# Luca96/carla-driving-rl-agent

Measured on AMD Instinct MI355X. Metric: PPO update-steps/sec (batch=256, 4x90x120x3 obs), higher is better.
Workload: dtype f32; 1 GPU; configs[1]: synthetic rollout buffer 256x4-frame 90x120x3 obs per GPU, full CARLANetwork fwd/bwd + PPO (re-sampled Beta, pathwise) / value loss + clip + Adam, fp32; per_gpu_batch=256, global_batch=256, parallelism=dp1, policy_loss=resampled (reference-faithful)

## Files before the change

carla-driving-rl-agent_amd/csrc/gemm_tn_lds.hip:

```cpp
#include <stdlib.h>

#include "colreduce.h"
#include "mfma_x3.h"

namespace cdrl {

struct TnLdsArgs {
    View A, D;
    float* part;
    int M, N, K, G, Mg;
    int rows_per, nspg;
    const float* a_stats;
    TnBnBwd db;
};

constexpr int TNL_R = 32;

template <int MODE, bool APRO, bool DPRO>
__global__ void __launch_bounds__(256, 2) tn_lds_kernel(TnLdsArgs a) {
    constexpr bool BH = MODE == 2, F32 = MODE == 0, X3 = MODE == 3;
    constexpr int NBUF = X3 ? 1 : 2, PL = X3 ? 3 : 1;
    constexpr int TNL_CS = F32 ? TNL_R + 1 : TNL_R / 2 + 1;
    __shared__ uint32_t AsT[NBUF * PL][128 * TNL_CS];
    __shared__ uint32_t DsT[NBUF * PL][128 * TNL_CS];
    constexpr uint32_t ESZ = BH ? 2u : 4u;
    const int tid = threadIdx.x, lane = tid & 63, wave = tid >> 6;
    const int l32 = lane & 31, lh = lane >> 5;
    const int K = a.K, N = a.N;
    const int k0 = blockIdx.y * 128, n0 = blockIdx.z * 128;
    const int KT = min(4, (K - k0 + 31) / 32), NT = min(4, (N - n0 + 31) / 32);
    const int grp = blockIdx.x / a.nspg;
    const int64_t gend = (int64_t)(grp + 1) * a.Mg;
    const int64_t mbeg64 = (int64_t)grp * a.Mg + (int64_t)(blockIdx.x % a.nspg) * a.rows_per;
    const int mb = (int)mbeg64;
    const int me = (int)min(mbeg64 + a.rows_per, gend);
    const int rg = tid >> 5, cq = tid & 31;
    const int ka = k0 + 4 * cq, nd = n0 + 4 * cq;
    float asc[4], ash[4], qm[4], qi[4], qsc[4], qsh[4], qk1[4], qk2[4], qk3[4];
#pragma unroll
    for (int j = 0; j < 4; ++j) {
        asc[j] = 1.0f;
        ash[j] = 0.0f;
        if (APRO) {
            const bool on = ka + j < K;
            asc[j] = on ? a.a_stats[2 * a.G * K + grp * K + ka + j] : 0.0f;
            ash[j] = on ? a.a_stats[3 * a.G * K + grp * K + ka + j] : 0.0f;
        }
        qm[j] = qi[j] = qsc[j] = qsh[j] = qk1[j] = qk2[j] = qk3[j] = 0.0f;
        if (DPRO && nd + j < N) {
            const int GN = a.G * N, o = grp * N + nd + j;
            qm[j] = a.db.stats[0 * GN + o];
            qi[j] = a.db.stats[1 * GN + o];
            qsc[j] = a.db.stats[2 * GN + o];
            qsh[j] = a.db.stats[3 * GN + o];
            qk1[j] = a.db.coef[0 * GN + o];
            qk2[j] = a.db.coef[1 * GN + o];
            qk3[j] = a.db.coef[2 * GN + o];
        }
    }
    const bool relu = DPRO && a.db.act == ACT_RELU6;
    const __amdgpu_buffer_rsrc_t rA = buffer_rsrc(a.A.p, (int)((int64_t)a.M * a.A.ld * ESZ));
    const __amdgpu_buffer_rsrc_t rD = buffer_rsrc(a.D.p, (int)((int64_t)a.M * a.D.ld * ESZ));
    const __amdgpu_buffer_rsrc_t rY = buffer_rsrc(DPRO ? a.db.y : a.D.p, (int)((int64_t)a.M * (DPRO ? N : a.D.ld) * ESZ));
    const bool a4 = (ka + 3 < K);
    const bool a2 = (ka + 1 < K);
    const bool d4 = (nd + 3 < N), d2 = (nd + 1 < N);
    const int shuf = DPRO ? a.db.shuffle_ctot : 0;
    uint32_t voA = a2 ? (uint32_t)(a.A.coff + ka) * ESZ : OOR;
    uint32_t voD0, voD1;
    const bool dhalf = shuf && d2 && !d4;
    if (shuf) {
        voD0 = d2 ? (uint32_t)(shuffle_dst(a.D.coff + nd, shuf) - (dhalf ? 1 : 0)) * ESZ : OOR;
        voD1 = d2 ? (uint32_t)(shuffle_dst(a.D.coff + nd + 1, shuf) - (dhalf ? 1 : 0)) * ESZ : OOR;
    } else {
        voD0 = d2 ? (uint32_t)(a.D.coff + nd) * ESZ : OOR;
        voD1 = d4 ? (uint32_t)(a.D.coff + nd + 2) * ESZ : OOR;
    }
    const uint32_t voY = d2 ? (uint32_t)nd * ESZ : OOR;
    const uint32_t sA = (uint32_t)a.A.ld * ESZ, sD = (uint32_t)a.D.ld * ESZ, sY = (uint32_t)N * ESZ;
    auto ld2 = [&](const __amdgpu_buffer_rsrc_t& rs, uint32_t vo, uint32_t ro, float& x0, float& x1) {
        const uint32_t off = (vo & OOR) ? OOR : vo + ro;
        if (BH) {
            const uint32_t w = __builtin_amdgcn_raw_buffer_load_b32(rs, off, 0, 0);
            x0 = bf_lo(w);
            x1 = bf_hi(w);
        } else {
            const u32x2_t w = __builtin_amdgcn_raw_buffer_load_b64(rs, off, 0, 0);
            x0 = __uint_as_float(w[0]);
            x1 = __uint_as_float(w[1]);
        }
    };
    struct Regs {
        float a[4][4], d[4][4], y[DPRO ? 4 : 1][DPRO ? 4 : 1];
    };
    auto load_chunk = [&](int m0, Regs& r) {
#pragma unroll
        for (int i = 0; i < 4; ++i) {
            const int m = m0 + 4 * rg + i;
            const uint32_t msk = m < me ? 0u : OOR;
            const uint32_t row = (uint32_t)m;
            ld2(rA, voA | msk, row * sA, r.a[i][0], r.a[i][1]);
            ld2(rA, (a4 ? voA + 2 * ESZ : OOR) | msk, row * sA, r.a[i][2], r.a[i][3]);
            if (shuf) {
                ld2(rD, voD0 | msk, row * sD, r.d[i][0], r.d[i][2]);
                ld2(rD, voD1 | msk, row * sD, r.d[i][1], r.d[i][3]);
                if (dhalf) {
                    r.d[i][0] = r.d[i][2];
                    r.d[i][1] = r.d[i][3];
                    r.d[i][2] = r.d[i][3] = 0.0f;
                }
            } else {
                ld2(rD, voD0 | msk, row * sD, r.d[i][0], r.d[i][1]);
                ld2(rD, voD1 | msk, row * sD, r.d[i][2], r.d[i][3]);
            }
            if (DPRO) {
                ld2(rY, voY | msk, row * sY, r.y[DPRO ? i : 0][0], r.y[DPRO ? i : 0][DPRO ? 1 : 0]);
                ld2(rY, (d4 ? voY + 2 * ESZ : OOR) | msk, row * sY, r.y[DPRO ? i : 0][DPRO ? 2 : 0], r.y[DPRO ? i : 0][DPRO ? 3 : 0]);
            }
        }
        __builtin_amdgcn_sched_barrier(0);
    };
    auto store_chunk = [&](int m0, int buf, const Regs& r) {
        float keep[4];
#pragma unroll
        for (int i = 0; i < 4; ++i) keep[i] = (m0 + 4 * rg + i) < me ? 1.0f : 0.0f;
#pragma unroll
        for (int j = 0; j < 4; ++j) {
            float x[4], d[4];
#pragma unroll
            for (int i = 0; i < 4; ++i) {
                x[i] = r.a[i][j];
                if (APRO) x[i] = fmaf(asc[j], x[i], ash[j]);
                d[i] = r.d[i][j];
                if (DPRO) {
                    const float y = r.y[DPRO ? i : 0][DPRO ? j : 0];
                    if (relu) {
                        const float z = fmaf(qsc[j], y, qsh[j]);
                        d[i] = relu6_open(z) ? d[i] : 0.0f;
                    }
                    const float xh = (y - qm[j]) * qi[j];
                    d[i] = keep[i] * (qk1[j] * (d[i] - qk2[j] - xh * qk3[j]));
                }
            }
            const int c = 4 * cq + j;
            if (F32) {
                uint32_t* pa = &AsT[buf][c * TNL_CS + 4 * rg];
                uint32_t* pd = &DsT[buf][c * TNL_CS + 4 * rg];
#pragma unroll
                for (int i = 0; i < 4; ++i) {
                    pa[i] = __float_as_uint(x[i]);
                    pd[i] = __float_as_uint(d[i]);
                }
            } else if (X3) {
#pragma unroll
                for (int pl = 0; pl < 3; ++pl) {
                    float hx[4], hd[4];
#pragma unroll
                    for (int i = 0; i < 4; ++i) {
                        hx[i] = (float)(bf16_t)x[i];
                        hd[i] = (float)(bf16_t)d[i];
                        x[i] -= hx[i];
                        d[i] -= hd[i];
                    }
                    uint32_t* pa = &AsT[pl][c * TNL_CS + 2 * rg];
                    pa[0] = bf_pack(hx[0], hx[1]);
                    pa[1] = bf_pack(hx[2], hx[3]);
                    uint32_t* pd = &DsT[pl][c * TNL_CS + 2 * rg];
                    pd[0] = bf_pack(hd[0], hd[1]);
                    pd[1] = bf_pack(hd[2], hd[3]);
                }
            } else {
                uint32_t* pa = &AsT[buf][c * TNL_CS + 2 * rg];
                pa[0] = bf_pack(x[0], x[1]);
                pa[1] = bf_pack(x[2], x[3]);
                uint32_t* pd = &DsT[buf][c * TNL_CS + 2 * rg];
                pd[0] = bf_pack(d[0], d[1]);
                pd[1] = bf_pack(d[2], d[3]);
            }
        }
    };
    f32x16 acc[4];
#pragma unroll
    for (int j = 0; j < 4; ++j)
#pragma unroll
        for (int q = 0; q < 16; ++q) acc[j][q] = 0.0f;
    auto frag = [&](const uint32_t* base, int col, int s) -> bf16x8 {
        const uint32_t* p = base + col * TNL_CS + 8 * s + 4 * lh;
        u32x4_t w;
        w[0] = p[0];
        w[1] = p[1];
        w[2] = p[2];
        w[3] = p[3];
        return __builtin_bit_cast(bf16x8, w);
    };
    auto mma_chunk = [&](int buf) {
        if (wave >= KT) return;
        if (F32) {
            const uint32_t* pa = &AsT[buf][(wave * 32 + l32) * TNL_CS + lh];
#pragma unroll
            for (int s = 0; s < TNL_R / 2; ++s) {
                const float av = __uint_as_float(pa[2 * s]);
#pragma unroll
                for (int j = 0; j < 4; ++j) {
                    if (j < NT) {
                        const float dv = __uint_as_float(DsT[buf][(j * 32 + l32) * TNL_CS + 2 * s + lh]);
                        acc[j] = __builtin_amdgcn_mfma_f32_32x32x2f32(av, dv, acc[j], 0, 0, 0);
                    }
                }
            }
            return;
        }
        if (X3) {
#pragma unroll
            for (int s = 0; s < TNL_R / 16; ++s) {
                const bf16x8 a1 = frag(AsT[0], wave * 32 + l32, s), a2 = frag(AsT[X3 ? 1 : 0], wave * 32 + l32, s),
                             a3 = frag(AsT[X3 ? 2 : 0], wave * 32 + l32, s);
#pragma unroll
                for (int j = 0; j < 4; ++j) {
                    if (j < NT) {
                        const bf16x8 d1 = frag(DsT[0], j * 32 + l32, s), d2 = frag(DsT[X3 ? 1 : 0], j * 32 + l32, s),
                                     d3 = frag(DsT[X3 ? 2 : 0], j * 32 + l32, s);
                        acc[j] = __builtin_amdgcn_mfma_f32_32x32x16_bf16(a2, d2, acc[j], 0, 0, 0);
                        acc[j] = __builtin_amdgcn_mfma_f32_32x32x16_bf16(a3, d1, acc[j], 0, 0, 0);
                        acc[j] = __builtin_amdgcn_mfma_f32_32x32x16_bf16(a1, d3, acc[j], 0, 0, 0);
                        acc[j] = __builtin_amdgcn_mfma_f32_32x32x16_bf16(a2, d1, acc[j], 0, 0, 0);
                        acc[j] = __builtin_amdgcn_mfma_f32_32x32x16_bf16(a1, d2, acc[j], 0, 0, 0);
                        acc[j] = __builtin_amdgcn_mfma_f32_32x32x16_bf16(a1, d1, acc[j], 0, 0, 0);
                    }
                }
            }
            return;
        }
#pragma unroll
        for (int s = 0; s < TNL_R / 16; ++s) {
            const bf16x8 af = frag(AsT[buf], wave * 32 + l32, s);
#pragma unroll
            for (int j = 0; j < 4; ++j) {
                if (j < NT) {
                    const bf16x8 df = frag(DsT[buf], j * 32 + l32, s);
                    acc[j] = __builtin_amdgcn_mfma_f32_32x32x16_bf16(af, df, acc[j], 0, 0, 0);
                }
            }
        }
    };
    Regs r0;
    int c = 0;
    if (mb < me) load_chunk(mb, r0);
    for (int m0 = mb; m0 < me; m0 += TNL_R, ++c) {
        store_chunk(m0, X3 ? 0 : (c & 1), r0);
        __syncthreads();
        if (m0 + TNL_R < me) load_chunk(m0 + TNL_R, r0);
        mma_chunk(X3 ? 0 : (c & 1));
        if (X3) __syncthreads();
    }
    if (wave >= KT) return;
    float* out = a.part + (int64_t)blockIdx.x * K * N;
#pragma unroll
    for (int j = 0; j < 4; ++j) {
        const int n = n0 + j * 32 + l32;
        if (j >= NT || n >= N) continue;
#pragma unroll
        for (int q = 0; q < 16; ++q) {
            const int kk = acc_row(k0 + wave * 32, q, lh);
            if (kk < K) out[(int64_t)kk * N + n] = acc[j][q];
        }
    }
}

struct TnlPlan {
    int gy, gz, nspg, nsplit, rows_per;
};

static TnlPlan tnl_plan(int M, int N, int K, int G) {
    TnlPlan p;
    p.gy = cdiv(K, 128);
    p.gz = cdiv(N, 128);
    const int Mg = M / G;
    static const int wgs = 384;
    int target = wgs / (p.gy * p.gz * G);
    if (target < 1) target = 1;
    int ns = Mg / 128;
    if (ns > target) ns = target;
    if (ns < 1) ns = 1;
    p.rows_per = cdiv(cdiv(Mg, ns), TNL_R) * TNL_R;
    p.nspg = cdiv(Mg, p.rows_per);
    p.nsplit = G * p.nspg;
    return p;
}

int64_t gemm_tn_lds_part_elems(int M, int N, int K, int G) { return (int64_t)tnl_plan(M, N, K, G).nsplit * K * N; }

bool gemm_tn_lds_supported(View A, View D, int N, int K, int shuffle_ctot) {
    if ((A.ld & 1) || (A.coff & 1) || (D.ld & 1) || (D.coff & 1) || (K & 1) || (N & 1)) return false;
    if (shuffle_ctot && ((shuffle_ctot >> 1) & 1)) return false;
    return true;
}

void gemm_tn_lds_plan(TnPlan& p, int M, int N, int K, int G, int shuffle_ctot) {
    const TnlPlan q = tnl_plan(M, N, K, G);
    p.kernel = 2;
    p.NJW = p.WK = p.NSPL = p.RS = p.RS2 = p.U = 0;
    p.gy = q.gy;
    p.gz = q.gz;
    p.nspg = q.nspg;
    p.nsplit = q.nsplit;
    p.rows_per = q.rows_per;
    p.part_slots = q.nsplit;
    p.dhalf = (p.dpro && shuffle_ctot && N % 4 == 2) ? 1 : 0;
}

int gemm_tn_lds(const TnPlan& p, View A, View D, float* Cout, int M, int N, int K, float* part, int accumulate, hipStream_t st, int G,
                const float* pro_stats, const TnBnBwd* dpro) {
    if (!p.ok || p.kernel != 2 || !gemm_tn_lds_supported(A, D, N, K, dpro ? dpro->shuffle_ctot : 0)) {
        set_error("gemm_tn_lds: not planned for this call (K=%d N=%d)", K, N);
        return -1;
    }
    TnLdsArgs a;
    a.A = A;
    a.D = D;
    a.part = part;
    a.M = M;
    a.N = N;
    a.K = K;
    a.G = G;
    a.Mg = M / G;
    a.rows_per = p.rows_per;
    a.nspg = p.nspg;
    a.a_stats = pro_stats;
    a.db = TnBnBwd{};
    if (dpro) a.db = *dpro;
    const dim3 grid(p.nsplit, p.gy, p.gz), blk(256);
    const bool ap = p.apro != 0, dp = p.dpro != 0;
#define CDRL_TNL(BHV)                                                                               \
    do {                                                                                            \
        if (ap && dp) hipLaunchKernelGGL((tn_lds_kernel<BHV, true, true>), grid, blk, 0, st, a);    \
        else if (ap) hipLaunchKernelGGL((tn_lds_kernel<BHV, true, false>), grid, blk, 0, st, a);    \
        else if (dp) hipLaunchKernelGGL((tn_lds_kernel<BHV, false, true>), grid, blk, 0, st, a);    \
        else hipLaunchKernelGGL((tn_lds_kernel<BHV, false, false>), grid, blk, 0, st, a);           \
    } while (0)
    switch (p.mode) {
        case 2: CDRL_TNL(2); break;
        case 3: CDRL_TNL(3); break;
        case 0: CDRL_TNL(0); break;
        default: CDRL_TNL(1); break;
    }
#undef CDRL_TNL
    CDRL_LAUNCH_CHECK();
    const int64_t n = (int64_t)K * N;
    return reduce_partials_f32(part, p.part_slots, n, n, Cout, accumulate, st);
}

}
```

Before: 79.51 update-steps/s.

## Store X3 split planes row-major in LDS and read via transpose fragment loads

For the 3-way bf16 split (X3) path of the TN GEMM, the LDS tiles switch from a column-major transposed layout to a row-major padded layout (stride 160 bf16). The store writes 8-byte vectors per row using a paired split helper, and the MMA reads fragments through a transposing LDS load helper. The aim is fewer, wider LDS stores with fewer bank conflicts and cheaper fragment fetches. It relies on the tr_frag helpers being correct for this layout, and the LDS footprint changes.

After: 78.46 update-steps/s. 1.3% lower.

```diff
diff --git a/carla-driving-rl-agent_amd/csrc/gemm_tn_lds.hip b/carla-driving-rl-agent_amd/csrc/gemm_tn_lds.hip
--- a/carla-driving-rl-agent_amd/csrc/gemm_tn_lds.hip
+++ b/carla-driving-rl-agent_amd/csrc/gemm_tn_lds.hip
@@ -21,10 +21,13 @@
     constexpr bool BH = MODE == 2, F32 = MODE == 0, X3 = MODE == 3;
     constexpr int NBUF = X3 ? 1 : 2, PL = X3 ? 3 : 1;
     constexpr int TNL_CS = F32 ? TNL_R + 1 : TNL_R / 2 + 1;
-    __shared__ uint32_t AsT[NBUF * PL][128 * TNL_CS];
-    __shared__ uint32_t DsT[NBUF * PL][128 * TNL_CS];
+    constexpr int LD = 160, LDW = LD / 2;
+    constexpr int PLW = X3 ? TNL_R * LDW : 128 * TNL_CS;
+    static_assert(!X3 || (LD % 4 == 0 && LD >= 128 && 2 * PL * PLW * 4 <= 64 * 1024), "8-byte lane addresses, 128 columns, two workgroups per CU");
+    __shared__ __attribute__((aligned(16))) uint32_t AsT[NBUF * PL][PLW];
+    __shared__ __attribute__((aligned(16))) uint32_t DsT[NBUF * PL][PLW];
     constexpr uint32_t ESZ = BH ? 2u : 4u;
-    const int tid = threadIdx.x, lane = tid & 63, wave = tid >> 6;
+    const int tid = threadIdx.x, lane = tid & 63, wave = X3 ? __builtin_amdgcn_readfirstlane(tid >> 6) : tid >> 6;
     const int l32 = lane & 31, lh = lane >> 5;
     const int K = a.K, N = a.N;
     const int k0 = blockIdx.y * 128, n0 = blockIdx.z * 128;
@@ -124,6 +127,40 @@
         float keep[4];
 #pragma unroll
         for (int i = 0; i < 4; ++i) keep[i] = (m0 + 4 * rg + i) < me ? 1.0f : 0.0f;
+        if constexpr (X3) {
+#pragma unroll
+            for (int i = 0; i < 4; ++i) {
+                float x[4], d[4];
+#pragma unroll
+                for (int j = 0; j < 4; ++j) {
+                    x[j] = r.a[i][j];
+                    if (APRO) x[j] = fmaf(asc[j], x[j], ash[j]);
+                    d[j] = r.d[i][j];
+                    if (DPRO) {
+                        const float y = r.y[DPRO ? i : 0][DPRO ? j : 0];
+                        if (relu) {
+                            const float z = fmaf(qsc[j], y, qsh[j]);
+                            d[j] = relu6_open(z) ? d[j] : 0.0f;
+                        }
+                        const float xh = (y - qm[j]) * qi[j];
+                        d[j] = keep[i] * (qk1[j] * (d[j] - qk2[j] - xh * qk3[j]));
+                    }
+                }
+                uint32_t ha[3][2], hd[3][2];
+#pragma unroll
+                for (int h = 0; h < 2; ++h) {
+                    x3_split2(f32x2{x[2 * h], x[2 * h + 1]}, ha[0][h], ha[1][h], ha[2][h]);
+                    x3_split2(f32x2{d[2 * h], d[2 * h + 1]}, hd[0][h], hd[1][h], hd[2][h]);
+                }
+                const int o = (4 * rg + i) * LDW + 2 * cq;
+#pragma unroll
+                for (int pl = 0; pl < 3; ++pl) {
+                    *reinterpret_cast<u32x2_t*>(&AsT[pl][o]) = u32x2_t{ha[pl][0], ha[pl][1]};
+                    *reinterpret_cast<u32x2_t*>(&DsT[pl][o]) = u32x2_t{hd[pl][0], hd[pl][1]};
+                }
+            }
+            return;
+        }
 #pragma unroll
         for (int j = 0; j < 4; ++j) {
             float x[4], d[4];
@@ -151,24 +188,6 @@
                     pa[i] = __float_as_uint(x[i]);
                     pd[i] = __float_as_uint(d[i]);
                 }
-            } else if (X3) {
-#pragma unroll
-                for (int pl = 0; pl < 3; ++pl) {
-                    float hx[4], hd[4];
-#pragma unroll
-                    for (int i = 0; i < 4; ++i) {
-                        hx[i] = (float)(bf16_t)x[i];
-                        hd[i] = (float)(bf16_t)d[i];
-                        x[i] -= hx[i];
-                        d[i] -= hd[i];
-                    }
-                    uint32_t* pa = &AsT[pl][c * TNL_CS + 2 * rg];
-                    pa[0] = bf_pack(hx[0], hx[1]);
-                    pa[1] = bf_pack(hx[2], hx[3]);
-                    uint32_t* pd = &DsT[pl][c * TNL_CS + 2 * rg];
-                    pd[0] = bf_pack(hd[0], hd[1]);
-                    pd[1] = bf_pack(hd[2], hd[3]);
-                }
             } else {
                 uint32_t* pa = &AsT[buf][c * TNL_CS + 2 * rg];
                 pa[0] = bf_pack(x[0], x[1]);
@@ -210,16 +229,19 @@
             }
             return;
         }
-        if (X3) {
+        if constexpr (X3) {
+            const __bf16* pa = reinterpret_cast<const __bf16*>(&AsT[0][0]) + wave * 32 + tr_frag_off(lane, LD);
+            const __bf16* pd = reinterpret_cast<const __bf16*>(&DsT[0][0]) + tr_frag_off(lane, LD);
+            constexpr int PLE = 2 * PLW;
 #pragma unroll
             for (int s = 0; s < TNL_R / 16; ++s) {
-                const bf16x8 a1 = frag(AsT[0], wave * 32 + l32, s), a2 = frag(AsT[X3 ? 1 : 0], wave * 32 + l32, s),
-                             a3 = frag(AsT[X3 ? 2 : 0], wave * 32 + l32, s);
+                const bf16x8 a1 = tr_frag<LD>(pa + 0 * PLE + 16 * s * LD), a2 = tr_frag<LD>(pa + 1 * PLE + 16 * s * LD),
+                             a3 = tr_frag<LD>(pa + 2 * PLE + 16 * s * LD);
 #pragma unroll
                 for (int j = 0; j < 4; ++j) {
                     if (j < NT) {
-                        const bf16x8 d1 = frag(DsT[0], j * 32 + l32, s), d2 = frag(DsT[X3 ? 1 : 0], j * 32 + l32, s),
-                                     d3 = frag(DsT[X3 ? 2 : 0], j * 32 + l32, s);
+                        const bf16x8 d1 = tr_frag<LD>(pd + 0 * PLE + 16 * s * LD + 32 * j), d2 = tr_frag<LD>(pd + 1 * PLE + 16 * s * LD + 32 * j),
+                                     d3 = tr_frag<LD>(pd + 2 * PLE + 16 * s * LD + 32 * j);
                         acc[j] = __builtin_amdgcn_mfma_f32_32x32x16_bf16(a2, d2, acc[j], 0, 0, 0);
                         acc[j] = __builtin_amdgcn_mfma_f32_32x32x16_bf16(a3, d1, acc[j], 0, 0, 0);
                         acc[j] = __builtin_amdgcn_mfma_f32_32x32x16_bf16(a1, d3, acc[j], 0, 0, 0);
```
